# willake/cpu-ray-tracer

Measured on AMD Instinct MI355X. Metric: Mrays/sec (primary+secondary), 1280x720 64spp path trace — pipelined throughput over 878 consecutive 64-spp windows of one progressive render (single_render = one such render alone), higher is better.
Workload: dtype f32; 1 GPU; bunny_scene.xml FileScene BVH-SAH path tracer, 1280x720, 64 spp/step (passes=1, depthLimit=5); 1 step = 64 frames = the next spp window of a progressive render; the 878 steps are one crt_render job (14 render kernel launch(es), a wavefront per (tile, 128 consecutive frames), + ordered accumulate), one sync at the end; triangles=4968, parallelism=tile-wave x1

## Files before the change

### cpu-ray-tracer_amd/__init__.py

```python
import ctypes as C
import os
import subprocess

import numpy as np

HERE = os.path.dirname(os.path.abspath(__file__))
REPO = os.path.dirname(HERE)
LIB_PATH = os.environ.get("CRT_LIB_PATH") or os.path.join(HERE, "libcrt_amd.so")

SCENE_FILE, SCENE_TLAS = 0, 1
UPDATE_TRANSFORMS, UPDATE_BOUNDS = 1, 2
ACCEL_KDTREE, ACCEL_GRID = 1, 2
KD_NODE_DTYPE = np.dtype([("aabbMin", "<f4", 3), ("left", "<i4"), ("aabbMax", "<f4", 3), ("right", "<i4"), ("splitDistance", "<f4"), ("splitAxis", "<i4"),
                          ("firstTri", "<u4"), ("triCount", "<u4")])


class CrtError(RuntimeError):
    def __init__(self, code, msg):
        super().__init__("crt error %d: %s" % (code, msg))
        self.code = code


class Config(C.Structure):
    _fields_ = [("width", C.c_int32), ("height", C.c_int32), ("depthLimit", C.c_int32), ("device", C.c_int32),
# ... 344 lines not shown
            raise ValueError("%s: O and D must be [N, 3] float32" % what)
        n = O.shape[0]
        if last_is_int:
            col = torch.zeros(n, dtype=torch.int32, device=dev) if last is None else torch.as_tensor(last, device=dev).to(torch.int32).expand(n)
            col = col.contiguous().view(torch.float32)
        else:
            col = torch.as_tensor(last, dtype=torch.float32, device=dev).reshape(-1).expand(n)
        return torch.cat([O, D, col.reshape(n, 1)], 1).contiguous()

    def find_nearest_device(self, rays=None, O=None, D=None, inside=None, accel=0, stream=None):
        import torch

        def run(st):
            r = self._records(rays, O, D, inside, True, "find_nearest_device")
            hits = torch.empty((r.shape[0], 7), dtype=torch.float32, device=r.device)
            self._ck(self.L.crt_find_nearest_device(self.h, int(accel), C.c_void_p(r.data_ptr()), C.c_void_p(hits.data_ptr()), C.c_size_t(r.shape[0]), C.c_void_p(st.cuda_stream)))
            return hits
        return self._enqueue(stream, run)

    def is_occluded_device(self, rays=None, O=None, D=None, t=None, accel=0, stream=None):
        import torch
        if rays is None and t is None:
            raise ValueError("is_occluded_device: t is required with O / D")

        def run(st):
            r = self._records(rays, O, D, t, False, "is_occluded_device")
            occ = torch.empty(r.shape[0], dtype=torch.int32, device=r.device)
            self._ck(self.L.crt_is_occluded_device(self.h, int(accel), C.c_void_p(r.data_ptr()), C.c_void_p(occ.data_ptr()), C.c_size_t(r.shape[0]), C.c_void_p(st.cuda_stream)))
            return occ
        return self._enqueue(stream, run)

    def get_hit_info_device(self, rays, hits, stream=None):
        import torch

        def run(st):
            r = self._records(rays, None, None, None, True, "get_hit_info_device")
            h = self._records(hits, None, None, None, True, "get_hit_info_device")
            if h.shape[0] != r.shape[0]:
                raise ValueError("get_hit_info_device: one hit record per ray")
            out = torch.empty((r.shape[0], 12), dtype=torch.float32, device=r.device)
            self._ck(self.L.crt_get_hit_info_device(self.h, C.c_void_p(r.data_ptr()), C.c_void_p(h.data_ptr()), C.c_void_p(out.data_ptr()), C.c_size_t(r.shape[0]), C.c_void_p(st.cuda_stream)))
            return out
        return self._enqueue(stream, run)

    def get_sky_color_device(self, rays=None, O=None, D=None, stream=None):
        import torch

        def run(st):
            r = self._records(rays, O, D, None, True, "get_sky_color_device")
            rgb = torch.empty((r.shape[0], 3), dtype=torch.float32, device=r.device)
            self._ck(self.L.crt_get_sky_color_device(self.h, C.c_void_p(r.data_ptr()), C.c_void_p(rgb.data_ptr()), C.c_size_t(r.shape[0]), C.c_void_p(st.cuda_stream)))
            return rgb
        return self._enqueue(stream, run)

    def _enqueue(self, stream, run):
        import torch
        st = stream if stream is not None else torch.cuda.current_stream(self.device)
        if st.cuda_stream != 0:
            with torch.cuda.stream(st):
                return run(st)
        side = getattr(self, "_side_stream", None)
        if side is None:
            side = self._side_stream = torch.cuda.Stream(device=self.device)
        side.wait_stream(st)
        with torch.cuda.stream(side):
            out = run(side)
        st.wait_stream(side)
        out.record_stream(st)
        return out

    def counters(self):
        c = CountersS()
        self._ck(self.L.crt_get_counters(self.h, C.byref(c)))
        return {n: int(getattr(c, n)) for n, _ in c._fields_}

    def reset_counters(self):
        self._ck(self.L.crt_reset_counters(self.h))

    def timing(self):
        t = TimingS()
        self._ck(self.L.crt_get_timing(self.h, C.byref(t)))
        return dict(render_kernel_ms=t.render_kernel_ms, resolve_kernel_ms=t.resolve_kernel_ms, render_launches=t.render_launches, pool_launches=t.pool_launches, split_launches=t.split_launches)

    def tile_clocks(self, tile_count):
        a = np.zeros((tile_count, 2), np.uint64)
        self._ck(self.L.crt_get_tile_clocks(self.h, _p(a)))
        return a

    def bind_accumulator(self, device_ptr):
        self._ck(self.L.crt_bind_accumulator(self.h, C.c_void_p(device_ptr)))

    def accumulator_device_ptr(self):
        p = C.c_void_p()
        self._ck(self.L.crt_accumulator_device_ptr(self.h, C.byref(p)))
        return p.value

def hit_fields(hits):
    import torch
    i = hits.view(torch.int32)
    return dict(t=hits[:, 0], u=hits[:, 1], v=hits[:, 2], objIdx=i[:, 3], triIdx=i[:, 4], traversed=i[:, 5], tested=i[:, 6])


def hit_info_fields(info):
    import torch
    return dict(I=info[:, 0:3], material=info.view(torch.int32)[:, 3], N=info[:, 4:7], u=info[:, 7], albedo=info[:, 8:11], v=info[:, 11])


class HostScene:

    def __init__(self, xml_path, kind, base_dir=None):
        self.L = lib()
        h = C.c_void_p()
        rc = self.L.crt_host_scene_load(xml_path.encode(), int(kind), (base_dir or "").encode(), C.byref(h))
        if rc != 0:
            raise CrtError(rc, self.L.crt_host_last_error().decode())
        self.h = h
        self.kind = int(kind)

    def close(self):
        if getattr(self, "h", None):
            self.L.crt_host_scene_free(self.h)
            self.h = None

    def __del__(self):
        try:
            self.close()
        except Exception:
            pass

    def _ck(self, rc):
        if rc != 0:
            raise CrtError(rc, self.L.crt_host_last_error().decode())

    def upload(self, ctx):
        self._ck(self.L.crt_host_scene_upload(self.h, ctx.h))

    def triangle_count(self):
        return self.L.crt_host_scene_triangle_count(self.h)

    def bvh_count(self):
        return self.L.crt_host_scene_bvh_count(self.h)

    def bvh(self, i=0):
        nu, tc, md = C.c_uint32(), C.c_uint32(), C.c_uint32()
        self._ck(self.L.crt_host_scene_bvh_info(self.h, i, C.byref(nu), C.byref(tc), C.byref(md)))
        nodes = np.zeros(nu.value, NODE_DTYPE)
        idx = np.zeros(tc.value, np.uint32)
        tris = np.zeros(tc.value, TRI_DTYPE)
        self._ck(self.L.crt_host_scene_bvh_copy(self.h, i, _p(nodes), _p(idx), _p(tris)))
        return dict(nodes=nodes, triIndices=idx, tris=tris, nodesUsed=nu.value, maxDepth=md.value)

    def move_and_refit(self, i, positions):
        positions = np.ascontiguousarray(positions, np.float32)
        self._ck(self.L.crt_host_scene_bvh_move_and_refit(self.h, int(i), _p(positions), C.c_uint32(positions.shape[0])))

    def build_alt(self, kind):
        self._ck(self.L.crt_host_scene_build_alt(self.h, int(kind)))
        if self.kind == 1:
            return [self.blas_alt(kind, i) for i in range(self.bvh_count())]
        return self._alt(kind, lambda info: self.L.crt_host_scene_alt_info(self.h, int(kind), info),
                         lambda a, b, c: self.L.crt_host_scene_alt_copy(self.h, int(kind), a, b, c))

    def blas_alt(self, kind, i):
        return self._alt(kind, lambda info: self.L.crt_host_scene_blas_alt_info(self.h, int(kind), int(i), info),
                         lambda a, b, c: self.L.crt_host_scene_blas_alt_copy(self.h, int(kind), int(i), a, b, c))

# ... 211 lines not shown
```

### cpu-ray-tracer_amd/csrc/device/render_pool.hip

```cpp
#include "dev_common.h"

namespace crt {

enum : uint32_t {
    F_OX = 0, F_OY, F_OZ, F_DX, F_DY, F_DZ,
    F_RX, F_RY, F_RZ,
    F_T,
    F_SEED, F_META,
    F_U, F_V,
    F_COUNT,
    F_CUR = F_U, F_PEND = F_V,
    F_TRI = F_RX
};
constexpr uint32_t kMetaItemMask = 0x7ffu, kMetaDepthShift = 11u, kMetaInside = 1u << 14, kMetaFresh = 1u << 15, kMetaObjShift = 16u, kMetaLowMask = 0xffffu;
constexpr uint32_t kQueueMask = 127u;

#ifndef CRT_POOL_MIN_WAVES
#define CRT_POOL_MIN_WAVES 4
#endif
#ifndef CRT_POOL_SHADE_MIN
#define CRT_POOL_SHADE_MIN 64
#endif
#ifndef CRT_POOL_NODE_STEPS
#define CRT_POOL_NODE_STEPS 2
#endif
#ifndef CRT_POOL_NODE2_MIN
#define CRT_POOL_NODE2_MIN 16
#endif
#ifndef CRT_POOL_STARVE
#define CRT_POOL_STARVE 40
#endif

#ifdef CRT_POOL_STAMPS
__device__ unsigned long long g_poolStamps[16];
#define CRT_PSTAMP(var) unsigned long long var; asm volatile("s_memtime %0\n\ts_waitcnt lgkmcnt(0)" : "=s"(var) :: "memory")
#define CRT_PACC(i, a, b) (pst[i] += (b) - (a))
#else
#define CRT_PSTAMP(var)
#define CRT_PACC(i, a, b)
#endif
#ifdef CRT_POOL_DENS
__device__ unsigned long long g_poolDens[32];
#define CRT_DENS(i, v) (dens[i] += (uint32_t)(v))
#define CRT_DENS_MASK(i, pred) (dens[i] += (uint32_t)__popcll(__builtin_amdgcn_ballot_w64(pred)))
#else
#define CRT_DENS(i, v)
#define CRT_DENS_MASK(i, pred)
#endif
#ifdef CRT_POOL_TIMELINE
__device__ unsigned long long* g_poolTimeline = nullptr;
#endif
__device__ __forceinline__ bool lane_in(uint64_t m) { return __builtin_amdgcn_inverse_ballot_w64(m); }
__device__ __forceinline__ uint64_t finite3_mask(f3 v)
{
    const uint32_t m = 0x7f800000u;
    return __builtin_amdgcn_ballot_w64((asu(v.x) & m) != m) & __builtin_amdgcn_ballot_w64((asu(v.y) & m) != m) & __builtin_amdgcn_ballot_w64((asu(v.z) & m) != m);
}
__device__ __forceinline__ uint32_t rank_in(uint64_t m) { return __builtin_amdgcn_mbcnt_hi((uint32_t)(m >> 32), __builtin_amdgcn_mbcnt_lo((uint32_t)m, 0u)); }

template <int KIND, bool COUNT, int S>
__global__ __launch_bounds__(64, CRT_POOL_MIN_WAVES) void render_pool_kernel(const Scene sc, float4* __restrict__ slab, float* __restrict__ facScratch, Counters* __restrict__ counters,
                                                             unsigned long long* __restrict__ tileClocks, const uint32_t* __restrict__ tileOrder,
                                                             uint32_t tileFirst, uint32_t tileStride, uint32_t tileCount, uint32_t tilesX,
                                                             uint32_t sppFirst, uint32_t frames, uint32_t passes, uint32_t groups, uint32_t rankFirst, uint32_t* __restrict__ tileCost, unsigned long long* __restrict__ launchClk)
{
    extern __shared__ uint32_t lds[];
    const uint32_t lane = threadIdx.x;
#ifdef CRT_POOL_TIMELINE
    const unsigned long long tl0 = wall_clock64();
#endif
    const unsigned long long clk0 = (COUNT || tileCost) ? wall_clock64() : 0ull;
    if (launchClk && lane == 0) { atomicMax(&launchClk[0], ~clk0); atomicMax(&launchClk[1], clk0); }
    const uint32_t rank0 = blockIdx.x / groups, grp = blockIdx.x - rank0 * groups, rank = rank0 + rankFirst;
    if (rank >= tileCount) return;
    const uint32_t tl = tileOrder ? tileOrder[rank] : rank;
    const uint32_t frame0 = grp * (uint32_t)S;
    const uint32_t nStreams = (frames - frame0 < (uint32_t)S) ? frames - frame0 : (uint32_t)S;
    const uint32_t tile = tileFirst + tl * tileStride;
    const uint32_t tx = tile % tilesX, ty = tile / tilesX;
    const char* __restrict__ geom = sc.geom;
    float* __restrict__ fac = facScratch + (size_t)blockIdx.x * (15u * (uint32_t)S);

    char* const ldsB = reinterpret_cast<char*>(lds);
    const uint32_t laneB = lane * 2u;
    uint32_t* st = lds + (sc.stackDepth + 1u) * 32u;
    float* stf = reinterpret_cast<float*>(st);
    uint8_t* qEnd = reinterpret_cast<uint8_t*>(st + F_COUNT * S);
    uint8_t* qBnc = qEnd + 128, * qRdy = qEnd + 256;
    auto stk_top = [&](uint32_t at) -> uint32_t { return *reinterpret_cast<const uint16_t*>(ldsB + at); };
    auto stk_put = [&](uint32_t at, uint32_t v) { *reinterpret_cast<uint16_t*>(ldsB + at) = (uint16_t)v; };

    Cnt cn; cn.rays = cn.primary = cn.interior = cn.leaf = cn.tri = cn.tlas = cn.visits = cn.meshhits = 0;
    uint32_t trips = 0;
#ifdef CRT_POOL_DENS
    uint32_t dens[32]; for (int i = 0; i < 32; i++) dens[i] = 0;
#endif
    const uint32_t items = 256u * passes;
    const uint32_t rowLen = 64u * passes;
    const f3 nil3 = mk3(0.0f, 0.0f, 0.0f);

    for (uint32_t s = lane; s < nStreams; s += 64u) {
        st[F_SEED * S + s] = init_seed(tx + ty * (uint32_t)sc.W + (sppFirst + (frame0 + s) * passes) * 1799u);
        st[F_META * S + s] = kMetaFresh;
        qEnd[s] = (uint8_t)s;
    }
    uint32_t endH = 0, endT = nStreams, bncH = 0, bncT = 0, rdyH = 0, rdyT = 0;

    uint64_t mRes = 0ull;
    uint64_t mFinite = ~0ull;
    uint32_t sid = 0, cur = kRefDone, spB = laneB, metaLo = 0u;
    f3 tO = nil3, tD = nil3, trD = nil3;
    Hit h; h.t = 1e34f; h.u = 0; h.v = 0; h.objIdx = -1; h.triIdx = -1;
    rec4 q0 = {0, 0, 0, 0}, q1 = q0, q2 = q0, q3 = q0;

    auto new_ray = [&](bool act, uint32_t s, f3 v, bool norm, f3 O, uint32_t seed, uint32_t meta) {
        f3 D = v, rD = v; Hit nh; nh.t = 1e34f; nh.u = 0; nh.v = 0; nh.objIdx = -1; nh.triIdx = -1;
        uint32_t ncur = kRefDone, pend = 0u;
        if (act) {
            const float inv = rcp_exact(__builtin_sqrtf(dot3(v, v)));
            D = norm ? v * inv : v;
            rD = rcp_exact3(D);
            cn.rays++;
            {
                const kernarg_f lp = scene_floats(offsetof(Scene, lightInvT));
                const kernarg_f ax = scene_floats(offsetof(Scene, lightAxis));
                LightFloor lf;
#pragma unroll
                for (int i = 0; i < 12; i++) lf.lightInvT[i] = lp[i];
                lf.lightSize = lp[15]; lf.floorN[0] = lp[19]; lf.floorN[1] = lp[20]; lf.floorN[2] = lp[21]; lf.floorD = lp[22];
                lf.lightAxis = asu(ax[0]); lf.floorAxisY = asu(ax[1]);
                hit_light_floor(lf, O, D, nh);
            }
            if (sc.rootIsPair) {
                const kernarg_f rp = scene_floats(offsetof(Scene, rootPair));
                const rec4 a0 = {rp[0], rp[1], rp[2], rp[3]}, a1 = {rp[4], rp[5], rp[6], rp[7]};
                const rec4 b0 = {rp[8], rp[9], rp[10], rp[11]}, b1 = {rp[12], rp[13], rp[14], rp[15]};
                float d1, d2;
                if (__builtin_amdgcn_ballot_w64(!finite3(rD)) == 0ull) { d1 = box_fast(a0, a1, O, rD, nh.t); d2 = box_fast(b0, b1, O, rD, nh.t); }
                else { d1 = box_exact(a0, a1, O, rD, nh.t); d2 = box_exact(b0, b1, O, rD, nh.t); }
                const bool sw = d1 > d2;
                const float dn = sw ? d2 : d1, df = sw ? d1 : d2;
                const uint32_t rn = sw ? asu(b1.w) : asu(a1.w), rf = sw ? asu(a1.w) : asu(b1.w);
                const bool hitN = dn != 1e30f;
                pend = (hitN && df != 1e30f) ? rf : 0u;
                ncur = hitN ? rn : kRefDone;
                if (COUNT) { if (KIND == 0) cn.interior++; else cn.tlas++; }
            } else ncur = sc.rootRef16;
            if (COUNT && KIND == 0 && (ncur & kRef16TagMask) == 0u && ncur != kRefDone) cn.leaf++;
            stf[F_OX * S + s] = O.x; stf[F_OY * S + s] = O.y; stf[F_OZ * S + s] = O.z;
            stf[F_DX * S + s] = D.x; stf[F_DY * S + s] = D.y; stf[F_DZ * S + s] = D.z;
            stf[F_RX * S + s] = rD.x; stf[F_RY * S + s] = rD.y; stf[F_RZ * S + s] = rD.z;
            stf[F_T * S + s] = nh.t;
            st[F_SEED * S + s] = seed; st[F_META * S + s] = meta | ((uint32_t)(nh.objIdx + 1) << kMetaObjShift);
            st[F_CUR * S + s] = ncur; st[F_PEND * S + s] = pend;
        }
        const uint32_t depth = (meta >> kMetaDepthShift) & 7u;
        const uint64_t mAct = __builtin_amdgcn_ballot_w64(act);
        const uint64_t mW = mAct & __builtin_amdgcn_ballot_w64(ncur != kRefDone);
        const uint64_t mStop = __builtin_amdgcn_ballot_w64((uint32_t)(nh.objIdx + 1) <= 1u) | __builtin_amdgcn_ballot_w64((int)depth >= sc.depthLimit);
        const uint64_t mE = mAct & ~mW & mStop, mB = mAct & ~mW & ~mStop;
        CRT_DENS(20, __popcll(mAct)); CRT_DENS(19, __popcll(mW));
        if (lane_in(mW)) qRdy[(rdyT + rank_in(mW)) & kQueueMask] = (uint8_t)s;
        if (lane_in(mE)) qEnd[(endT + rank_in(mE)) & kQueueMask] = (uint8_t)s;
        if (lane_in(mB)) qBnc[(bncT + rank_in(mB)) & kQueueMask] = (uint8_t)s;
        rdyT += (uint32_t)__popcll(mW); endT += (uint32_t)__popcll(mE); bncT += (uint32_t)__popcll(mB);
    };
    auto world_ray = [&]() {
        tO = mk3(stf[F_OX * S + sid], stf[F_OY * S + sid], stf[F_OZ * S + sid]);
        tD = mk3(stf[F_DX * S + sid], stf[F_DY * S + sid], stf[F_DZ * S + sid]);
        trD = mk3(stf[F_RX * S + sid], stf[F_RY * S + sid], stf[F_RZ * S + sid]);
    };

    uint64_t mNode2 = 0ull;
    auto node_step = [&](uint64_t m) {
        const bool allFinite = (m & ~mFinite) == 0ull;
        if (lane_in(m)) {
            if (COUNT) { if (KIND == 1 && (cur & kRef16TlasBit) != 0u) cn.tlas++; else cn.interior++; }
            const uint32_t top = stk_top(spB);
            float d1, d2;
            if (__builtin_expect(allFinite, 1)) { d1 = box_fast(q0, q1, tO, trD, h.t); d2 = box_fast(q2, q3, tO, trD, h.t); }
            else { d1 = box_exact(q0, q1, tO, trD, h.t); d2 = box_exact(q2, q3, tO, trD, h.t); }
            const bool sw = d1 > d2;
            const float dn = sw ? d2 : d1, df = sw ? d1 : d2;
            const uint32_t rn = sw ? asu(q3.w) : asu(q1.w), rf = sw ? asu(q1.w) : asu(q3.w);
            stk_put(spB + 128u, rf);
            const bool hitN = dn != 1e30f, push = hitN && df != 1e30f;
            const bool pop = !hitN && spB != laneB;
            cur = hitN ? rn : (pop ? top : kRefDone);
            spB = spB + (push ? 128u : 0u) - (pop ? 128u : 0u);
            if (COUNT && (cur & kRef16TagMask) == 0u && cur != kRefDone) cn.leaf++;
        }
    };
    auto load_records = [&](uint64_t m) {
        const uint32_t idx = cur & kRef16IndexMask;
        const bool inter = (cur & kRef16Interior) != 0u;
        uint32_t oa = idx * (inter ? 64u : 48u) + (inter ? 0u : sc.leafOff - 48u);
        if (KIND == 1 && (cur & kRef16TlasBit) != 0u)
            oa = (cur & kRef16Interior) ? sc.instOff + idx * 128u : sc.tlasPairOff + idx * 64u;
        if (lane_in(m)) { q0 = ldg(geom, oa); q1 = ldg(geom, oa + 16u); q2 = ldg(geom, oa + 32u); q3 = ldg(geom, oa + 48u); }
    };

    auto tri_step = [&](uint64_t m) {
        CRT_DENS(3, 1); CRT_DENS(4, __popcll(m));
        if (lane_in(m)) {
            if (COUNT) cn.tri++;
            const uint32_t top = stk_top(spB);
            hit_tri(q0, q1, q2, tO, tD, h);
            const bool more = asu(q2.w) > 1u;
            const bool pop = !more && spB != laneB;
            const uint32_t next = more ? cur + 1u : (pop ? top : kRefDone);
            spB -= pop ? 128u : 0u;
            if (COUNT && !more && (next & kRef16TagMask) == 0u && next != kRefDone) cn.leaf++;
            cur = next;
        }
    };

#ifdef CRT_POOL_STAMPS
    unsigned long long pst[12] = {0, 0, 0, 0, 0, 0, 0, 0, 0, 0, 0, 0};
#endif
    for (;;) {
        CRT_PSTAMP(p0);
        if (mRes != 0ull) {
            uint64_t mNode, mTlas = 0ull;
            if (KIND == 0) mNode = mRes & __builtin_amdgcn_ballot_w64(cur > 0x7fffu);
            else { mTlas = mRes & __builtin_amdgcn_ballot_w64(cur >= kRef16TlasLeaf); mNode = mRes & __builtin_amdgcn_ballot_w64(cur - kRef16TlasBit < 0x8000u); }
            const uint64_t mTri = mRes & ~(mNode | mTlas);
            asm volatile("" : "+v"(q0), "+v"(q1), "+v"(q2), "+v"(q3));
            CRT_DENS(22, __popcll(mRes));
            if (mNode) { CRT_DENS(1, 1); CRT_DENS(2, __popcll(mNode)); }

            if (KIND == 1 && mTlas) { CRT_DENS(23, 1); CRT_DENS(24, __popcll(mTlas)); }
            uint64_t mBack = 0ull;
            if (KIND == 1 && mTlas != 0ull) {
                if (lane_in(mTlas)) {
                    if (COUNT) { cn.tlas++; cn.visits++; }
                    const f3 O = mk3(stf[F_OX * S + sid], stf[F_OY * S + sid], stf[F_OZ * S + sid]);
                    const f3 D = mk3(stf[F_DX * S + sid], stf[F_DY * S + sid], stf[F_DZ * S + sid]);
                    to_object_space(q0, q1, q2, O, D, tO, tD, trD);
                    spB += 128u; stk_put(spB, kRef16Return);
                    const uint32_t next = asu(q3.y);
                    if (COUNT && (next & kRef16TagMask) == 0u && next != kRefDone) cn.leaf++;
                    cur = next;
                }
                mFinite = (mFinite & ~mTlas) | (mTlas & finite3_mask(trD));
            }
            if (mNode != 0ull) node_step(mNode);
#if CRT_POOL_NODE_STEPS > 1
            uint64_t mLeafNow = 0ull;
#pragma unroll
            for (int rep = 1; rep < CRT_POOL_NODE_STEPS; rep++) {
                const uint64_t mStepped = rep == 1 ? mNode : mNode2;
                mNode2 = mStepped & (KIND == 0 ? __builtin_amdgcn_ballot_w64(cur > 0x7fffu) : __builtin_amdgcn_ballot_w64(cur - kRef16TlasBit < 0x8000u));
                if ((uint32_t)__popcll(mNode2) < (uint32_t)CRT_POOL_NODE2_MIN) { mNode2 = 0ull; break; }
                const uint64_t mLeaf = mStepped & __builtin_amdgcn_ballot_w64((cur & kRef16TagMask) == 0u) & ~__builtin_amdgcn_ballot_w64(cur == kRefDone);
                load_records(mNode2 | mLeaf);
                mLeafNow |= mLeaf;
                CRT_DENS(28, 1); CRT_DENS(29, __popcll(mNode2));
                node_step(mNode2);
            }
            const uint64_t mTriAll = mTri | mLeafNow;
            const uint64_t mTriRan = mTriAll;
#else
            const uint64_t mTriAll = mTri;
            const uint64_t mTriRan = mTriAll;
#endif
            if (mTriAll != 0ull) tri_step(mTriAll);
            if (KIND == 1) {
                mBack = (mNode | mTriRan) & __builtin_amdgcn_ballot_w64(cur == kRef16Return);
                if (mBack != 0ull) {
                    if (lane_in(mBack)) {
                        world_ray();
                        const bool pop = spB != laneB;
                        const uint32_t top = stk_top(spB);
                        cur = pop ? top : kRefDone; spB -= pop ? 128u : 0u;
                        if (COUNT && (cur & kRef16TagMask) == 0u && cur != kRefDone) cn.leaf++;
                    }
                    mFinite = (mFinite & ~mBack) | (mBack & finite3_mask(trD));
                }
            }
            asm volatile("" ::: "memory");
            const uint64_t mFin = mRes & __builtin_amdgcn_ballot_w64(cur == kRefDone);
            if (mFin != 0ull) {
                CRT_DENS(5, 1); CRT_DENS(6, __popcll(mFin));
                const uint32_t depth = (metaLo >> kMetaDepthShift) & 7u;
                const uint64_t mStop = __builtin_amdgcn_ballot_w64((uint32_t)(h.objIdx + 1) <= 1u) | __builtin_amdgcn_ballot_w64((int)depth >= sc.depthLimit);
                const uint64_t mE = mFin & mStop, mB = mFin & ~mStop;
                if (lane_in(mFin)) {
                    stf[F_T * S + sid] = h.t; stf[F_U * S + sid] = h.u; stf[F_V * S + sid] = h.v;
                    st[F_TRI * S + sid] = (uint32_t)h.triIdx;
                    st[F_META * S + sid] = metaLo | ((uint32_t)(h.objIdx + 1) << kMetaObjShift);
                }
                if (lane_in(mE)) qEnd[(endT + rank_in(mE)) & kQueueMask] = (uint8_t)sid;
                if (lane_in(mB)) qBnc[(bncT + rank_in(mB)) & kQueueMask] = (uint8_t)sid;
                endT += (uint32_t)__popcll(mE); bncT += (uint32_t)__popcll(mB);
                mRes &= ~mFin;
            }
            asm volatile("" ::: "memory");
        }
        CRT_PSTAMP(p1); CRT_PACC(0, p0, p1);
        if (__builtin_expect(mRes == 0ull, 0)) {
            if ((endT - endH) + (bncT - bncH) + (rdyT - rdyH) == 0u) break;
        }
        if (COUNT) trips++;
        CRT_DENS(0, 1);
        {
            const uint32_t nRdy = rdyT - rdyH;
            const uint64_t mFree = ~mRes;
            if (nRdy != 0u) if (mFree != 0ull) {
                const uint32_t myRank = rank_in(mFree);
                const uint64_t mTake = mFree & __builtin_amdgcn_ballot_w64(myRank < nRdy);
                CRT_DENS(7, 1); CRT_DENS(8, __popcll(mTake));
                if (lane_in(mTake)) {
                    sid = qRdy[(rdyH + myRank) & kQueueMask];
                    tO = mk3(stf[F_OX * S + sid], stf[F_OY * S + sid], stf[F_OZ * S + sid]);
                    tD = mk3(stf[F_DX * S + sid], stf[F_DY * S + sid], stf[F_DZ * S + sid]);
                    trD = mk3(stf[F_RX * S + sid], stf[F_RY * S + sid], stf[F_RZ * S + sid]);
                    const uint32_t meta = st[F_META * S + sid];
                    h.t = stf[F_T * S + sid]; h.objIdx = (int)(meta >> kMetaObjShift) - 1; h.u = 0; h.v = 0; h.triIdx = -1;
                    metaLo = meta & kMetaLowMask;
                    cur = st[F_CUR * S + sid];
                    const uint32_t pend = st[F_PEND * S + sid];
                    stk_put(laneB + 128u, pend);
                    spB = laneB + (pend ? 128u : 0u);
                }
                mFinite = (mFinite & ~mTake) | (mTake & finite3_mask(trD));
                mRes |= mTake;
                rdyH += (uint32_t)__popcll(mTake);
            }
            if (mRes != 0ull) {
                CRT_DENS(21, 1);
                const uint32_t idx = cur & kRef16IndexMask;
                const bool inter = (cur & kRef16Interior) != 0u;
                uint32_t oa = idx * (inter ? 64u : 48u) + (inter ? 0u : sc.leafOff - 48u);
                if (KIND == 1 && (cur & kRef16TlasBit) != 0u)
                    oa = (cur & kRef16Interior) ? sc.instOff + idx * 128u : sc.tlasPairOff + idx * 64u;
                if (!lane_in(mRes)) oa = 0u;
                q0 = ldg(geom, oa); q1 = ldg(geom, oa + 16u); q2 = ldg(geom, oa + 32u); q3 = ldg(geom, oa + 48u);
            }
        }
        asm volatile("" ::: "memory");
        {
            const uint32_t nEnd = endT - endH, nBnc = bncT - bncH, nRdy = rdyT - rdyH, nRes = (uint32_t)__popcll(mRes);
            const bool starving = nRes + nRdy < (uint32_t)CRT_POOL_STARVE;
            bool runEnd = false, runBnc = false;
            if ((nEnd | nBnc) >= (uint32_t)CRT_POOL_SHADE_MIN || starving) {
                runEnd = nEnd >= (uint32_t)CRT_POOL_SHADE_MIN || (starving && nEnd > 0u && nEnd >= nBnc);
                runBnc = nBnc >= (uint32_t)CRT_POOL_SHADE_MIN || (starving && nBnc > nEnd);
            }

            CRT_PSTAMP(p2b); CRT_PACC(1, p1, p2b);
            if (runEnd) {
                const uint32_t n = nEnd < 64u ? nEnd : 64u;
                const bool act = lane < n;
                const uint32_t s = act ? qEnd[(endH + lane) & kQueueMask] : 0u;
                endH += n;
                uint32_t meta = 0, seed = 0; int obj = -1; f3 D = nil3;
                if (act) { meta = st[F_META * S + s]; seed = st[F_SEED * S + s]; obj = (int)(meta >> kMetaObjShift) - 1; D = mk3(stf[F_DX * S + s], stf[F_DY * S + s], stf[F_DZ * S + s]); }
                const bool first = (meta & kMetaFresh) != 0u;
                const int depth = (int)((meta >> kMetaDepthShift) & 7u);
                uint32_t item = meta & kMetaItemMask;
                const bool ended = act && !first, miss = ended && obj == -1;
                CRT_DENS(9, 1); CRT_DENS(10, n); CRT_DENS_MASK(11, miss); CRT_DENS_MASK(13, act && first); CRT_DENS_MASK(25, ended && depth > 0); CRT_DENS_MASK(26, ended && depth > 1); CRT_DENS_MASK(27, ended && depth > 2);
                if (ended && obj >= 2) cn.meshhits++;
                float fk[15];
#pragma unroll
                for (int k = 0; k < 5; k++) {
                    fk[3 * k] = fk[3 * k + 1] = fk[3 * k + 2] = 0.0f;
                    if (ended && depth > k) {
#pragma unroll
                        for (int j = 0; j < 3; j++) fk[3 * k + j] = __hip_atomic_load(fac + (3 * k + j) * S + s, __ATOMIC_RELAXED, __HIP_MEMORY_SCOPE_AGENT);
                    }
                }
                uint32_t skyTexel = 0u;
                if (miss) {
                    const float phi = crt_atan2f(-D.z, D.x) + CRT_PI, theta = crt_acosf(-D.y);
                    const kernarg_f sk = scene_floats(offsetof(Scene, skyOffset));
                    skyTexel = sc.texels[tex_index(asu(sk[0]), (int)asu(sk[1]), (int)asu(sk[2]), phi * CRT_INV2PI, theta * CRT_INVPI)];
                }
                bool gen = act && first;
                size_t sampleAt = 0;
                if (ended) {
                    uint32_t pix = item, pass = 0;
                    if (passes != 1u) { pix = item / passes; pass = item - pix * passes; }
                    const uint32_t fr = frame0 + s;
                    sampleAt = (((size_t)(fr >> 6) * tileCount + tl) * 256u + pix) * rowLen + ((fr & 63u) * passes + pass);
                    item++;
                    gen = item < items;
                }
                const kernarg_f cam = scene_floats(offsetof(Scene, camPos));
                const f3 camPos = mk3(cam[0], cam[1], cam[2]);
                f3 v = camPos;
                if (gen) {
                    const uint32_t pix = (passes == 1u) ? item : item / passes;
                    const int x = (int)(tx * 16u + (pix & 15u)), y = (int)(ty * 16u + (pix >> 4));
                    const float jy = rnd(seed);
                    const float jx = rnd(seed);
                    const float u = ((float)x + jx) * cam[12], vv = ((float)y + jy) * cam[13];
                    const f3 TL = mk3(cam[3], cam[4], cam[5]), TR = mk3(cam[6], cam[7], cam[8]), BL = mk3(cam[9], cam[10], cam[11]);
                    const f3 P = TL + u * (TR - TL) + vv * (BL - TL);
                    v = P - camPos;
                    cn.primary++;
                }
                CRT_DENS_MASK(12, gen);
                CRT_PSTAMP(e1); CRT_PACC(2, p2b, e1);
                new_ray(gen, s, v, true, camPos, seed, item);
                CRT_PSTAMP(e2); CRT_PACC(3, e1, e2);
                if (ended) {
                    f3 L = miss ? tex_unpack(skyTexel) : ((depth >= sc.depthLimit) ? mk3(0, 0, 0) : mk3(24, 24, 22));
#pragma unroll
                    for (int k = 4; k >= 0; k--)
                        if (depth > k) L = mk3(fk[3 * k], fk[3 * k + 1], fk[3 * k + 2]) * L;
                    slab[sampleAt] = make_float4(L.x, L.y, L.z, 0.0f);
                }
#ifdef CRT_POOL_STAMPS
                { CRT_PSTAMP(e3); CRT_PACC(4, e2, e3); pst[10]++; }
#endif
                asm volatile("" :: "v"(fk[0]), "v"(fk[1]), "v"(fk[2]), "v"(fk[3]), "v"(fk[4]), "v"(fk[5]), "v"(fk[6]), "v"(fk[7]), "v"(fk[8]), "v"(fk[9]), "v"(fk[10]), "v"(fk[11]), "v"(fk[12]), "v"(fk[13]), "v"(fk[14]), "v"(skyTexel));
            }
            CRT_PSTAMP(p3);
            asm volatile("" ::: "memory");
            if (runBnc) {
                const uint32_t n = nBnc < 64u ? nBnc : 64u;
                const bool act = lane < n;
                const uint32_t s = act ? qBnc[(bncH + lane) & kQueueMask] : 0u;
                bncH += n;
                f3 O = nil3, D = nil3; float ht = 0, hu = 0, hv = 0; int obj = 1; uint32_t tri = 0, seed = 0, meta = 0;
                if (act) {
                    tri = st[F_TRI * S + s];
                    O = mk3(stf[F_OX * S + s], stf[F_OY * S + s], stf[F_OZ * S + s]);
                    D = mk3(stf[F_DX * S + s], stf[F_DY * S + s], stf[F_DZ * S + s]);
                    ht = stf[F_T * S + s]; hu = stf[F_U * S + s]; hv = stf[F_V * S + s];
                    seed = st[F_SEED * S + s]; meta = st[F_META * S + s]; obj = (int)(meta >> kMetaObjShift) - 1;
                }
                const bool mesh = act && obj >= 2;
                CRT_DENS(14, 1); CRT_DENS(15, n); CRT_DENS_MASK(16, mesh);
                rec4 s0 = {0, 0, 0, 0}, s1 = s0, s2 = s0, s3 = s0;
                if (mesh) { const uint32_t so = sc.shadeOff + tri * 64u; s0 = ldg(geom, so); s1 = ldg(geom, so + 16u); s2 = ldg(geom, so + 32u); s3 = ldg(geom, so + 48u); cn.meshhits++; }
                const bool inside = (meta & kMetaInside) != 0u;
                const int depth = (int)((meta >> kMetaDepthShift) & 7u);
                const uint32_t item = meta & kMetaItemMask;
                float tu = 0, tv = 0; uint32_t tOff = 0; int tW = 0, tH = 0;
                f3 I = O, N = O, absorb = O; float refl = 0, refr = 0;
                f3 v = O, pre = O; bool norm = false, diffuse = false, newInside = false;
                if (act) {
                    I = O + ht * D;
                    if (obj == 1) {
                        const kernarg_f fl = scene_floats(offsetof(Scene, floorN));
                        const kernarg_f fm = scene_floats(offsetof(Scene, floorMat));
                        N = mk3(fl[0], fl[1], fl[2]);
                        if (N.y == 1) {
                            float u = I.x, vv = I.z;
                            u *= fl[4]; vv *= fl[4];
                            tu = u - __builtin_floorf(u); tv = vv - __builtin_floorf(vv);
                        }
                        refl = fm[0]; refr = fm[1];
                        absorb = mk3(fm[2], fm[3], fm[4]);
                        tOff = asu(fm[5]); tW = (int)asu(fm[6]); tH = (int)asu(fm[7]);
                    } else {
                        const f3 n0 = mk3(s0.x, s0.y, s0.z), n1 = mk3(s0.w, s1.x, s1.y), n2 = mk3(s1.z, s1.w, s2.x);
                        const float w = 1 - hu - hv;
                        const f3 Nn = w * n0 + hu * n1 + hv * n2;
                        tu = w * s2.y + hu * s2.w + hv * s3.y;
                        tv = w * s2.z + hu * s3.x + hv * s3.z;
                        const rec4* mp = reinterpret_cast<const rec4*>(sc.mats + (int)asu(s3.w));
                        const rec4 m0 = mp[0], m1 = mp[1];
                        refl = m0.x; refr = m0.y; absorb = mk3(m0.z, m0.w, m1.x);
                        tOff = asu(m1.y); tW = (int)asu(m1.z); tH = (int)asu(m1.w);
                        if (KIND == 0) {
                            N = normalize3(Nn);
                        } else {
                            const uint32_t io = sc.instOff + (uint32_t)(obj - 2) * 128u + 64u;
                            const rec4 r0 = ldg(geom, io), r1 = ldg(geom, io + 16), r2 = ldg(geom, io + 32);
                            N = normalize3(mk3(r0.x * Nn.x + r0.y * Nn.y + r0.z * Nn.z + r0.w * 0.0f,
                                               r1.x * Nn.x + r1.y * Nn.y + r1.z * Nn.z + r1.w * 0.0f,
                                               r2.x * Nn.x + r2.y * Nn.y + r2.z * Nn.z + r2.w * 0.0f));
                        }
                    }
                    if (dot3(N, D) > 0) N = -N;
                    uint32_t texel = 0x00ffffffu;
                    if (tW > 0) texel = sc.texels[tex_index(tOff, tW, tH, tu, tv)];
                    f3 medium = mk3(1, 1, 1);
                    if (inside) {
                        const f3 ab = absorb * -ht;
                        medium = mk3(crt_expf(ab.x), crt_expf(ab.y), crt_expf(ab.z));
                    }
                    CRT_PSTAMP(b1); CRT_PACC(5, p3, b1);
                    const float r = rnd(seed);
                    const bool mirror = r < refl, dielectric = !mirror && r < refl + refr;
                    if (mirror) {
                        v = D - 2.0f * N * dot3(N, D);
                    } else if (dielectric) {
                        v = D - 2.0f * N * dot3(N, D);
                        const float n1 = inside ? 1.2f : 1, n2 = inside ? 1 : 1.2f;
                        const float eta = n1 / n2, cosi = dot3(-D, N);
                        const float cost2 = 1.0f - eta * eta * (1 - cosi * cosi);
                        if (cost2 > 0) {
                            const float a = n1 - n2, b2 = n1 + n2, R0 = (a * a) / (b2 * b2), cc = 1 - cosi;
                            const float Fr = R0 + (1 - R0) * (cc * cc * cc * cc * cc);
                            const f3 T = eta * D + ((eta * cosi - __builtin_sqrtf(__builtin_fabsf(cost2))) * N);
                            if (rnd(seed) > Fr) { v = T; newInside = !inside; }
                        }
                    } else {
                        f3 Rr;
                        do {
                            const float rz = rnd_pm1(seed);
                            const float ry = rnd_pm1(seed);
                            const float rx = rnd_pm1(seed);
                            Rr = mk3(rx, ry, rz);
                        } while (dot3(Rr, Rr) > 1);
                        if (dot3(Rr, N) < 0) Rr = Rr * -1.0f;
                        v = Rr; norm = true; diffuse = true;
                    }
                    const f3 c = (tW > 0) ? tex_unpack(texel) : mk3(1.0f, 1.0f, 1.0f);
                    if (diffuse) {
                        const f3 brdf = c * CRT_INVPI;
                        pre = medium * brdf * 2.0f * CRT_PI;
                    } else pre = c * medium;
                    CRT_PSTAMP(b2); CRT_PACC(6, b1, b2);
                    const float inv = rcp_exact(__builtin_sqrtf(dot3(v, v)));
                    const f3 nv = norm ? v * inv : v;
                    v = nv;
                    const f3 factor = diffuse ? pre * dot3(nv, N) : pre;
                    float* fd = fac + (3 * depth) * S + s;
                    __hip_atomic_store(fd, factor.x, __ATOMIC_RELAXED, __HIP_MEMORY_SCOPE_AGENT);
                    __hip_atomic_store(fd + S, factor.y, __ATOMIC_RELAXED, __HIP_MEMORY_SCOPE_AGENT);
                    __hip_atomic_store(fd + 2 * S, factor.z, __ATOMIC_RELAXED, __HIP_MEMORY_SCOPE_AGENT);
                    O = I + nv * CRT_EPS;
                    CRT_PSTAMP(b3); CRT_PACC(7, b2, b3);
                }
                CRT_PSTAMP(b4);
                new_ray(act, s, v, false, O, seed, item | ((uint32_t)(depth + 1) << kMetaDepthShift) | (newInside ? kMetaInside : 0u));
#ifdef CRT_POOL_STAMPS
                { CRT_PSTAMP(b5); CRT_PACC(8, b4, b5); pst[11]++; }
#endif
                asm volatile("" :: "v"(s0), "v"(s1), "v"(s2), "v"(s3));
            }
#ifdef CRT_POOL_STAMPS
            pst[9]++;
#endif
        }
    }
#ifdef CRT_POOL_STAMPS
    if (lane == 0) for (int i = 0; i < 12; i++) atomicAdd(&g_poolStamps[i], pst[i]);
#endif
#ifdef CRT_POOL_DENS
    if (lane == 0) for (int i = 0; i < 32; i++) if (dens[i]) atomicAdd(&g_poolDens[i], (unsigned long long)dens[i]);
#endif

#ifdef CRT_POOL_TIMELINE
    if (lane == 0 && g_poolTimeline) { uint32_t hw; asm volatile("s_getreg_b32 %0, hwreg(HW_REG_HW_ID)" : "=s"(hw)); g_poolTimeline[3 * (size_t)blockIdx.x] = tl0; g_poolTimeline[3 * (size_t)blockIdx.x + 1] = wall_clock64(); g_poolTimeline[3 * (size_t)blockIdx.x + 2] = hw; }
#endif
    if (tileCost && lane == 0 && nStreams == (uint32_t)S) atomicMax(&tileCost[tl], (uint32_t)((wall_clock64() - clk0) * 64ull / (uint32_t)S));
    if (launchClk && lane == 0) { const unsigned long long now = wall_clock64(), last = __hip_atomic_load(&launchClk[1], __ATOMIC_RELAXED, __HIP_MEMORY_SCOPE_AGENT), from = last > clk0 ? last : clk0; if (now > from) atomicAdd(&launchClk[2], now - from); }
    if (COUNT && tileClocks && lane == 0 && groups == 1u) {
        tileClocks[2 * tl] = wall_clock64() - clk0;
        tileClocks[2 * tl + 1] = trips;
    }
    uint32_t vals[8] = {cn.rays, cn.primary, cn.interior, cn.leaf, cn.tri, cn.tlas, cn.visits, cn.meshhits};
#pragma unroll
    for (int i = 0; i < 8; i++) {
        if (!COUNT && i >= 2 && i != 7) continue;
        uint32_t sum = wave_sum(vals[i]);
        if (lane == 0 && sum) atomicAdd(&counters->v[i], (unsigned long long)sum);
    }
}

}

#ifndef CRT_POOL_STREAMS
#define CRT_POOL_STREAMS 128
#endif
extern "C" uint32_t crt_pool_streams(uint32_t frames) { return frames > 64u ? (uint32_t)CRT_POOL_STREAMS : 64u; }
#ifndef CRT_POOL_EXTRA_LDS
#define CRT_POOL_EXTRA_LDS 0
#endif
extern "C" uint32_t crt_pool_lds_bytes(uint32_t stackDepth, uint32_t streams) { return (stackDepth + 1u) * 64u * 2u + crt::F_COUNT * streams * 4u + 3u * 128u + (uint32_t)CRT_POOL_EXTRA_LDS; }
extern "C" size_t crt_pool_scratch_bytes_per_window(uint32_t tileCount) { return (size_t)tileCount * 128u * 15u * 4u; }

#ifdef CRT_POOL_STAMPS
extern "C" int crt_debug_pool_stamps(unsigned long long* out, int reset)
{
    if (out && hipMemcpyFromSymbol(out, HIP_SYMBOL(crt::g_poolStamps), 128) != hipSuccess) return -1;
    if (reset) { unsigned long long z[16] = {}; if (hipMemcpyToSymbol(HIP_SYMBOL(crt::g_poolStamps), z, 128) != hipSuccess) return -1; }
    return 0;
}
#endif
#ifdef CRT_POOL_DENS
extern "C" int crt_debug_pool_density(unsigned long long* out, int reset)
{
    if (out && hipMemcpyFromSymbol(out, HIP_SYMBOL(crt::g_poolDens), 256) != hipSuccess) return -1;
    if (reset) { unsigned long long z[32] = {}; if (hipMemcpyToSymbol(HIP_SYMBOL(crt::g_poolDens), z, 256) != hipSuccess) return -1; }
    return 0;
}
#endif
#ifdef CRT_POOL_TIMELINE
static unsigned long long* g_timelineHost = nullptr; static size_t g_timelineCount = 0;
extern "C" size_t crt_debug_pool_timeline(unsigned long long* out, size_t cap)
{
    const size_t n = g_timelineCount < cap ? g_timelineCount : cap;
    if (out && n) (void)hipMemcpy(out, g_timelineHost, n * 24, hipMemcpyDeviceToHost);
    return g_timelineCount;
}
#endif
extern "C" hipError_t crt_launch_render_pool(const crt::Scene* sc, void* slab, void* facScratch, crt::Counters* counters, unsigned long long* tileClocks, const uint32_t* tileOrder,
                                             uint32_t tileFirst, uint32_t tileStride, uint32_t tileCount, uint32_t tilesX, uint32_t sppFirst,
                                             uint32_t frames, uint32_t passes, int collectStats, uint32_t rankFirst, uint32_t* tileCost, unsigned long long* launchClk, hipStream_t stream)
{
    if (tileCount == 0 || frames == 0) return hipSuccess;
    if (!sc->ref16ok) return hipErrorInvalidValue;
    const uint32_t S = crt_pool_streams(frames);
    const uint32_t groups = (frames + S - 1u) / S;
    if ((unsigned long long)tileCount * groups > 0x7fffffffull) return hipErrorInvalidValue;
    if (rankFirst >= tileCount) return hipSuccess;
    dim3 grid((tileCount - rankFirst) * groups), block(64);
#ifdef CRT_POOL_TIMELINE
    { static unsigned long long* buf = nullptr; static size_t cap = 0;
      if (cap < (size_t)grid.x) { if (buf) (void)hipFree(buf); (void)hipMalloc((void**)&buf, (size_t)grid.x * 24); cap = grid.x; (void)hipMemcpyToSymbol(HIP_SYMBOL(crt::g_poolTimeline), &buf, sizeof(buf)); }
      (void)hipMemsetAsync(buf, 0, (size_t)grid.x * 24, stream); g_timelineHost = buf; g_timelineCount = grid.x; }
#endif
    const uint32_t ldsBytes = crt_pool_lds_bytes(sc->stackDepth, S);
#define CRT_LAUNCH(K, C, SS) hipLaunchKernelGGL((crt::render_pool_kernel<K, C, SS>), grid, block, ldsBytes, stream, *sc, (float4*)slab, (float*)facScratch, counters, tileClocks, tileOrder, tileFirst, tileStride, tileCount, tilesX, sppFirst, frames, passes, groups, rankFirst, tileCost, launchClk)
#define CRT_LAUNCH_S(K, C) do { if (S == 64u) CRT_LAUNCH(K, C, 64); else CRT_LAUNCH(K, C, CRT_POOL_STREAMS); } while (0)
    if (sc->kind == 0) { if (collectStats) CRT_LAUNCH_S(0, true); else CRT_LAUNCH_S(0, false); }
    else { if (collectStats) CRT_LAUNCH_S(1, true); else CRT_LAUNCH_S(1, false); }
#undef CRT_LAUNCH_S
#undef CRT_LAUNCH
    return hipGetLastError();
}
```

Measured before the change: 29820 Mrays/s.

## Add direct sky-only prologue that resolves all-miss primary samples before pool loop

Before entering the wavefront queue machinery, each wave generates its primary rays in lockstep and tests them only against the light/floor and the two root boxes. While every lane misses everything, it writes the sky texel directly to the slab and moves to the next item. It hands over to the normal pool loop with the item counter advanced once any lane hits. This skips the queue/LDS bookkeeping for tiles that see only sky, at the cost of extra register pressure, duplicated work on the first hitting item, and more code in the kernel.

```diff
diff --git a/cpu-ray-tracer_amd/__init__.py b/cpu-ray-tracer_amd/__init__.py
--- a/cpu-ray-tracer_amd/__init__.py
+++ b/cpu-ray-tracer_amd/__init__.py
@@ -450,6 +450,13 @@
         self._ck(self.L.crt_get_timing(self.h, C.byref(t)))
         return dict(render_kernel_ms=t.render_kernel_ms, resolve_kernel_ms=t.resolve_kernel_ms, render_launches=t.render_launches, pool_launches=t.pool_launches, split_launches=t.split_launches)
 
+    def pool_direct_stats(self, reset=False):
+        self.sync()
+        out = (C.c_uint64 * 3)()
+        if self.L.crt_debug_pool_direct(out, C.c_int(int(reset))) != 0:
+            raise CrtError(-2, "crt_debug_pool_direct failed")
+        return dict(finished_waves=int(out[0]), handed_over_waves=int(out[1]), direct_samples=int(out[2]))
+
     def tile_clocks(self, tile_count):
         a = np.zeros((tile_count, 2), np.uint64)
         self._ck(self.L.crt_get_tile_clocks(self.h, _p(a)))
diff --git a/cpu-ray-tracer_amd/csrc/device/render_pool.hip b/cpu-ray-tracer_amd/csrc/device/render_pool.hip
--- a/cpu-ray-tracer_amd/csrc/device/render_pool.hip
+++ b/cpu-ray-tracer_amd/csrc/device/render_pool.hip
@@ -18,6 +18,9 @@
 #ifndef CRT_POOL_MIN_WAVES
 #define CRT_POOL_MIN_WAVES 4
 #endif
+#ifndef CRT_POOL_DIRECT
+#define CRT_POOL_DIRECT 1
+#endif
 #ifndef CRT_POOL_SHADE_MIN
 #define CRT_POOL_SHADE_MIN 64
 #endif
@@ -57,6 +60,54 @@
     return __builtin_amdgcn_ballot_w64((asu(v.x) & m) != m) & __builtin_amdgcn_ballot_w64((asu(v.y) & m) != m) & __builtin_amdgcn_ballot_w64((asu(v.z) & m) != m);
 }
 __device__ __forceinline__ uint32_t rank_in(uint64_t m) { return __builtin_amdgcn_mbcnt_hi((uint32_t)(m >> 32), __builtin_amdgcn_mbcnt_lo((uint32_t)m, 0u)); }
+
+template <class Words> __device__ __forceinline__ f3 primary_dir(Words cam, uint32_t tx, uint32_t ty, uint32_t pix, uint32_t& seed)
+{
+    const int x = (int)(tx * 16u + (pix & 15u)), y = (int)(ty * 16u + (pix >> 4));
+    const float jy = rnd(seed);
+    const float jx = rnd(seed);
+    const float u = ((float)x + jx) * cam[12], vv = ((float)y + jy) * cam[13];
+    const f3 camPos = mk3(cam[0], cam[1], cam[2]);
+    const f3 TL = mk3(cam[3], cam[4], cam[5]), TR = mk3(cam[6], cam[7], cam[8]), BL = mk3(cam[9], cam[10], cam[11]);
+    const f3 P = TL + u * (TR - TL) + vv * (BL - TL);
+    return P - camPos;
+}
+template <class Words> __device__ __forceinline__ void light_floor_step(Words lp, Words ax, f3 O, f3 D, Hit& nh)
+{
+    LightFloor lf;
+#pragma unroll
+    for (int i = 0; i < 12; i++) lf.lightInvT[i] = lp[i];
+    lf.lightSize = lp[15]; lf.floorN[0] = lp[19]; lf.floorN[1] = lp[20]; lf.floorN[2] = lp[21]; lf.floorD = lp[22];
+    lf.lightAxis = asu(ax[0]); lf.floorAxisY = asu(ax[1]);
+    hit_light_floor(lf, O, D, nh);
+}
+template <class Words> __device__ __forceinline__ void root_step(Words rp, f3 O, f3 rD, float t, uint32_t& ncur, uint32_t& pend)
+{
+    const rec4 a0 = {rp[0], rp[1], rp[2], rp[3]}, a1 = {rp[4], rp[5], rp[6], rp[7]};
+    const rec4 b0 = {rp[8], rp[9], rp[10], rp[11]}, b1 = {rp[12], rp[13], rp[14], rp[15]};
+    float d1, d2;
+    if (__builtin_amdgcn_ballot_w64(!finite3(rD)) == 0ull) { d1 = box_fast(a0, a1, O, rD, t); d2 = box_fast(b0, b1, O, rD, t); }
+    else { d1 = box_exact(a0, a1, O, rD, t); d2 = box_exact(b0, b1, O, rD, t); }
+    const bool sw = d1 > d2;
+    const float dn = sw ? d2 : d1, df = sw ? d1 : d2;
+    const uint32_t rn = sw ? asu(b1.w) : asu(a1.w), rf = sw ? asu(a1.w) : asu(b1.w);
+    const bool hitN = dn != 1e30f;
+    pend = (hitN && df != 1e30f) ? rf : 0u;
+    ncur = hitN ? rn : kRefDone;
+}
+template <class Words> __device__ __forceinline__ uint32_t sky_texel_index(Words sk, f3 D)
+{
+    const float phi = crt_atan2f(-D.z, D.x) + CRT_PI, theta = crt_acosf(-D.y);
+    return tex_index(asu(sk[0]), (int)asu(sk[1]), (int)asu(sk[2]), phi * CRT_INV2PI, theta * CRT_INVPI);
+}
+__device__ __forceinline__ size_t sample_address(uint32_t fr, uint32_t tileCount, uint32_t tl, uint32_t pix, uint32_t pass, uint32_t passes, uint32_t rowLen)
+{
+    return (((size_t)(fr >> 6) * tileCount + tl) * 256u + pix) * rowLen + ((fr & 63u) * passes + pass);
+}
+
+#if CRT_POOL_DIRECT
+__device__ unsigned long long g_poolDirect[3];
+#endif
 
 template <int KIND, bool COUNT, int S>
 __global__ __launch_bounds__(64, CRT_POOL_MIN_WAVES) void render_pool_kernel(const Scene sc, float4* __restrict__ slab, float* __restrict__ facScratch, Counters* __restrict__ counters,
@@ -99,12 +150,103 @@
     const uint32_t rowLen = 64u * passes;
     const f3 nil3 = mk3(0.0f, 0.0f, 0.0f);
 
+#ifdef CRT_POOL_STAMPS
+    unsigned long long pst[13] = {0, 0, 0, 0, 0, 0, 0, 0, 0, 0, 0, 0, 0};
+#endif
+    CRT_PSTAMP(d0);
+#if CRT_POOL_DIRECT
+    constexpr int kSlots = S / 64;
+    uint32_t dSeed[kSlots]; bool dAct[kSlots];
+#pragma unroll
+    for (int j = 0; j < kSlots; j++) {
+        const uint32_t s = lane + 64u * (uint32_t)j;
+        dAct[j] = s < nStreams;
+        dSeed[j] = init_seed(tx + ty * (uint32_t)sc.W + (sppFirst + (frame0 + s) * passes) * 1799u);
+    }
+    uint32_t dItem = 0;
+    if (sc.rootIsPair) {
+        float cam[14], lp[23], ax[2], rp[16], sk[3];
+        {
+            const kernarg_f kc = scene_floats(offsetof(Scene, camPos)), kl = scene_floats(offsetof(Scene, lightInvT)), ka = scene_floats(offsetof(Scene, lightAxis));
+            const kernarg_f kr = scene_floats(offsetof(Scene, rootPair)), ks = scene_floats(offsetof(Scene, skyOffset));
+#pragma unroll
+            for (int i = 0; i < 14; i++) cam[i] = kc[i];
+#pragma unroll
+            for (int i = 0; i < 23; i++) lp[i] = kl[i];
+#pragma unroll
+            for (int i = 0; i < 16; i++) rp[i] = kr[i];
+            ax[0] = ka[0]; ax[1] = ka[1]; sk[0] = ks[0]; sk[1] = ks[1]; sk[2] = ks[2];
+        }
+        const f3 camPos = mk3(cam[0], cam[1], cam[2]);
+        uint32_t pix = 0, pass = 0, pendPix = 0, pendPass = 0;
+        uint32_t texel[kSlots]; bool pending = false;
+#pragma unroll
+        for (int j = 0; j < kSlots; j++) texel[j] = 0u;
+        for (;;) {
+            bool clean = dItem < items;
+            f3 D[kSlots]; uint32_t seedAfter[kSlots];
+#pragma unroll
+            for (int j = 0; j < kSlots; j++) { D[j] = nil3; seedAfter[j] = dSeed[j]; }
+            if (clean) {
+#pragma unroll
+                for (int j = 0; j < kSlots; j++) {
+                    if (j > 0 && nStreams <= 64u * (uint32_t)j) break;
+                    bool hitAny = false;
+                    if (dAct[j]) {
+                        const f3 v = primary_dir((const float*)cam, tx, ty, pix, seedAfter[j]);
+                        const float inv = rcp_exact(__builtin_sqrtf(dot3(v, v)));
+                        D[j] = v * inv;
+                        const f3 rD = rcp_exact3(D[j]);
+                        Hit nh; nh.t = 1e34f; nh.u = 0; nh.v = 0; nh.objIdx = -1; nh.triIdx = -1;
+                        light_floor_step((const float*)lp, (const float*)ax, camPos, D[j], nh);
+                        uint32_t ncur, pend;
+                        root_step((const float*)rp, camPos, rD, nh.t, ncur, pend);
+                        hitAny = nh.objIdx != -1 || ncur != kRefDone;
+                    }
+                    clean = clean && __builtin_amdgcn_ballot_w64(hitAny) == 0ull;
+                }
+            }
+            if (pending) {
+#pragma unroll
+                for (int j = 0; j < kSlots; j++)
+                    if (dAct[j]) {
+                        const f3 L = tex_unpack(texel[j]);
+                        slab[sample_address(frame0 + lane + 64u * (uint32_t)j, tileCount, tl, pendPix, pendPass, passes, rowLen)] = make_float4(L.x, L.y, L.z, 0.0f);
+                    }
+            }
+            if (!clean) break;
+#pragma unroll
+            for (int j = 0; j < kSlots; j++) {
+                if (dAct[j]) texel[j] = sc.texels[sky_texel_index((const float*)sk, D[j])];
+                dSeed[j] = seedAfter[j];
+            }
+            CRT_DENS(30, 1);
+            pending = true; pendPix = pix; pendPass = pass;
+            dItem++;
+            if (++pass == passes) { pass = 0; pix++; }
+        }
+#pragma unroll
+        for (int j = 0; j < kSlots; j++)
+            if (dAct[j]) { cn.rays += dItem; cn.primary += dItem; if (COUNT) { if (KIND == 0) cn.interior += dItem; else cn.tlas += dItem; } }
+    }
+    const bool handOver = dItem < items;
+    CRT_PSTAMP(d1); CRT_PACC(12, d0, d1);
+    if (handOver) CRT_DENS(31, 1);
+    if (COUNT && lane == 0) { atomicAdd(&g_poolDirect[handOver ? 1 : 0], 1ull); if (dItem) atomicAdd(&g_poolDirect[2], (unsigned long long)dItem * nStreams); }
+#pragma unroll
+    for (int j = 0; j < kSlots; j++) {
+        const uint32_t s = lane + 64u * (uint32_t)j;
+        if (handOver && dAct[j]) { st[F_SEED * S + s] = dSeed[j]; st[F_META * S + s] = kMetaFresh | dItem; qEnd[s] = (uint8_t)s; }
+    }
+    uint32_t endH = 0, endT = handOver ? nStreams : 0u, bncH = 0, bncT = 0, rdyH = 0, rdyT = 0;
+#else
     for (uint32_t s = lane; s < nStreams; s += 64u) {
         st[F_SEED * S + s] = init_seed(tx + ty * (uint32_t)sc.W + (sppFirst + (frame0 + s) * passes) * 1799u);
         st[F_META * S + s] = kMetaFresh;
         qEnd[s] = (uint8_t)s;
     }
     uint32_t endH = 0, endT = nStreams, bncH = 0, bncT = 0, rdyH = 0, rdyT = 0;
+#endif
 
     uint64_t mRes = 0ull;
     uint64_t mFinite = ~0ull;
@@ -121,29 +263,9 @@
             D = norm ? v * inv : v;
             rD = rcp_exact3(D);
             cn.rays++;
-            {
-                const kernarg_f lp = scene_floats(offsetof(Scene, lightInvT));
-                const kernarg_f ax = scene_floats(offsetof(Scene, lightAxis));
-                LightFloor lf;
-#pragma unroll
-                for (int i = 0; i < 12; i++) lf.lightInvT[i] = lp[i];
-                lf.lightSize = lp[15]; lf.floorN[0] = lp[19]; lf.floorN[1] = lp[20]; lf.floorN[2] = lp[21]; lf.floorD = lp[22];
-                lf.lightAxis = asu(ax[0]); lf.floorAxisY = asu(ax[1]);
-                hit_light_floor(lf, O, D, nh);
-            }
+            light_floor_step(scene_floats(offsetof(Scene, lightInvT)), scene_floats(offsetof(Scene, lightAxis)), O, D, nh);
             if (sc.rootIsPair) {
-                const kernarg_f rp = scene_floats(offsetof(Scene, rootPair));
-                const rec4 a0 = {rp[0], rp[1], rp[2], rp[3]}, a1 = {rp[4], rp[5], rp[6], rp[7]};
-                const rec4 b0 = {rp[8], rp[9], rp[10], rp[11]}, b1 = {rp[12], rp[13], rp[14], rp[15]};
-                float d1, d2;
-                if (__builtin_amdgcn_ballot_w64(!finite3(rD)) == 0ull) { d1 = box_fast(a0, a1, O, rD, nh.t); d2 = box_fast(b0, b1, O, rD, nh.t); }
-                else { d1 = box_exact(a0, a1, O, rD, nh.t); d2 = box_exact(b0, b1, O, rD, nh.t); }
-                const bool sw = d1 > d2;
-                const float dn = sw ? d2 : d1, df = sw ? d1 : d2;
-                const uint32_t rn = sw ? asu(b1.w) : asu(a1.w), rf = sw ? asu(a1.w) : asu(b1.w);
-                const bool hitN = dn != 1e30f;
-                pend = (hitN && df != 1e30f) ? rf : 0u;
-                ncur = hitN ? rn : kRefDone;
+                root_step(scene_floats(offsetof(Scene, rootPair)), O, rD, nh.t, ncur, pend);
                 if (COUNT) { if (KIND == 0) cn.interior++; else cn.tlas++; }
             } else ncur = sc.rootRef16;
             if (COUNT && KIND == 0 && (ncur & kRef16TagMask) == 0u && ncur != kRefDone) cn.leaf++;
@@ -215,9 +337,6 @@
         }
     };
 
-#ifdef CRT_POOL_STAMPS
-    unsigned long long pst[12] = {0, 0, 0, 0, 0, 0, 0, 0, 0, 0, 0, 0};
-#endif
     for (;;) {
         CRT_PSTAMP(p0);
         if (mRes != 0ull) {
@@ -372,18 +491,13 @@
                     }
                 }
                 uint32_t skyTexel = 0u;
-                if (miss) {
-                    const float phi = crt_atan2f(-D.z, D.x) + CRT_PI, theta = crt_acosf(-D.y);
-                    const kernarg_f sk = scene_floats(offsetof(Scene, skyOffset));
-                    skyTexel = sc.texels[tex_index(asu(sk[0]), (int)asu(sk[1]), (int)asu(sk[2]), phi * CRT_INV2PI, theta * CRT_INVPI)];
-                }
+                if (miss) skyTexel = sc.texels[sky_texel_index(scene_floats(offsetof(Scene, skyOffset)), D)];
                 bool gen = act && first;
                 size_t sampleAt = 0;
                 if (ended) {
                     uint32_t pix = item, pass = 0;
                     if (passes != 1u) { pix = item / passes; pass = item - pix * passes; }
-                    const uint32_t fr = frame0 + s;
-                    sampleAt = (((size_t)(fr >> 6) * tileCount + tl) * 256u + pix) * rowLen + ((fr & 63u) * passes + pass);
+                    sampleAt = sample_address(frame0 + s, tileCount, tl, pix, pass, passes, rowLen);
                     item++;
                     gen = item < items;
                 }
@@ -392,13 +506,7 @@
                 f3 v = camPos;
                 if (gen) {
                     const uint32_t pix = (passes == 1u) ? item : item / passes;
-                    const int x = (int)(tx * 16u + (pix & 15u)), y = (int)(ty * 16u + (pix >> 4));
-                    const float jy = rnd(seed);
-                    const float jx = rnd(seed);
-                    const float u = ((float)x + jx) * cam[12], vv = ((float)y + jy) * cam[13];
-                    const f3 TL = mk3(cam[3], cam[4], cam[5]), TR = mk3(cam[6], cam[7], cam[8]), BL = mk3(cam[9], cam[10], cam[11]);
-                    const f3 P = TL + u * (TR - TL) + vv * (BL - TL);
-                    v = P - camPos;
+                    v = primary_dir(cam, tx, ty, pix, seed);
                     cn.primary++;
                 }
                 CRT_DENS_MASK(12, gen);
@@ -541,7 +649,7 @@
         }
     }
 #ifdef CRT_POOL_STAMPS
-    if (lane == 0) for (int i = 0; i < 12; i++) atomicAdd(&g_poolStamps[i], pst[i]);
+    if (lane == 0) for (int i = 0; i < 13; i++) atomicAdd(&g_poolStamps[i], pst[i]);
 #endif
 #ifdef CRT_POOL_DENS
     if (lane == 0) for (int i = 0; i < 32; i++) if (dens[i]) atomicAdd(&g_poolDens[i], (unsigned long long)dens[i]);
@@ -577,6 +685,16 @@
 extern "C" uint32_t crt_pool_lds_bytes(uint32_t stackDepth, uint32_t streams) { return (stackDepth + 1u) * 64u * 2u + crt::F_COUNT * streams * 4u + 3u * 128u + (uint32_t)CRT_POOL_EXTRA_LDS; }
 extern "C" size_t crt_pool_scratch_bytes_per_window(uint32_t tileCount) { return (size_t)tileCount * 128u * 15u * 4u; }
 
+extern "C" int crt_debug_pool_direct(unsigned long long* out, int reset)
+{
+#if CRT_POOL_DIRECT
+    if (out && hipMemcpyFromSymbol(out, HIP_SYMBOL(crt::g_poolDirect), 24) != hipSuccess) return -1;
+    if (reset) { unsigned long long z[3] = {}; if (hipMemcpyToSymbol(HIP_SYMBOL(crt::g_poolDirect), z, 24) != hipSuccess) return -1; }
+#else
+    if (out) out[0] = out[1] = out[2] = 0ull;
+#endif
+    return 0;
+}
 #ifdef CRT_POOL_STAMPS
 extern "C" int crt_debug_pool_stamps(unsigned long long* out, int reset)
 {
```

Result: slower. 29340 Mrays/s (-1.6%).
